# TXH-mercury/VALOR

Hardware: AMD Instinct MI355X
Metric: pretrain samples/sec (V+A+T clip) (higher is better)
Workload: dtype bf16

## Files before the change

### valor_amd/csrc/gemm8.hip

```cpp
#include "gemm_common.h"
#include <stdlib.h>

#define HT_BYTES 16384
#define BUF_BYTES (4 * HT_BYTES)
#define OFF_A0 0
#define OFF_A1 HT_BYTES
#define OFF_B0 (2 * HT_BYTES)
#define OFF_B1 (3 * HT_BYTES)

DEVINL bf16x8_t read_frag_tr8(const char* img, int off, int kk) {
    const char* a = img + off + kk * (32 * 256);
    s16x4_t lo = lds_read_tr4(a), hi = lds_read_tr4(a + 4 * 256);
    return __builtin_bit_cast(bf16x8_t, __builtin_shufflevector(lo, hi, 0, 1, 2, 3, 4, 5, 6, 7));
}

template <bool TA, bool TB, bool ASMTR, bool NTS = false, int SCHED = 0>
__global__ __launch_bounds__(512, 2) void gemm_8ph_kernel(GemmArgs p) {
    typedef bf16_t T;
    constexpr int BK = 64;
    extern __shared__ __attribute__((aligned(16))) char smem[];

    const int tid = threadIdx.x;
    const int lane = tid & 63;
    const int wave = __builtin_amdgcn_readfirstlane(tid >> 6);
    const int wm = wave >> 2, wn = wave & 3;
    const int fr = lane & 15, fg = lane >> 4;

    const int tiles_n = (p.N + 255) >> 8;
    const int tiles_m = (p.M + 255) >> 8;
    int logical, slice = 0;
    if (p.kslices > 1) {
        const int ntiles = tiles_m * tiles_n;
        const int item = xcd_remap(blockIdx.x, ntiles * p.kslices);
        slice = item / ntiles;
        logical = item - slice * ntiles;
    } else {
        logical = xcd_remap(blockIdx.x, tiles_m * tiles_n);
    }
    int tm = logical / tiles_n, tn = logical - tm * tiles_n;
    if (p.raster_g > 0 && p.kslices <= 1) {
        const int G = p.raster_g, per = G * tiles_m;
        const int grp = logical / per, w = logical - grp * per;
        const int gw = min(G, tiles_n - grp * G);
        tm = w / gw;
        tn = grp * G + (w - tm * gw);
    }
    const int m0 = tm << 8, n0 = tn << 8;

    const int nk_total = p.K / BK;
    int ks_begin = 0, ks_end = nk_total;
    if (p.kslices > 1) {
        ks_begin = slice * p.ksteps_per_slice;
        ks_end = ks_begin + p.ksteps_per_slice;
        if (ks_end > nk_total) ks_end = nk_total;
        if (ks_begin > nk_total) ks_begin = nk_total;
    }
    const int k_first = ks_begin * BK;

    f32x4_t acc[8][4];
#pragma unroll
    for (int i = 0; i < 8; ++i)
#pragma unroll
        for (int j = 0; j < 4; ++j) acc[i][j] = (f32x4_t){0.f, 0.f, 0.f, 0.f};

    const bool do_rs = TA && p.rowsum_out != nullptr && tn == 0;
    f32x4_t racc[2] = {(f32x4_t){0.f, 0.f, 0.f, 0.f}, (f32x4_t){0.f, 0.f, 0.f, 0.f}};
    const bf16x8_t ones = __builtin_bit_cast(bf16x8_t, (u32x4_t){0x3f803f80u, 0x3f803f80u, 0x3f803f80u, 0x3f803f80u});

    const rsrc_t rsA = make_rsrc(p.A, p.bytesA), rsB = make_rsrc(p.B, p.bytesB);
    int voA[2][2], voB[2][2];
    int stepA, stepB;
    {
        const int ldA_b = (int)(p.lda * 2), ldB_b = (int)(p.ldb * 2);
#pragma unroll
        for (int hf = 0; hf < 2; ++hf)
#pragma unroll
            for (int i = 0; i < 2; ++i) {
                const int pc = wave * 2 + i;
                if constexpr (!TA) {
                    const int r = pc * 8 + (lane >> 3), c = (lane & 7) ^ ((lane >> 3) & 7);
                    const int trow = hf * 128 + r;
                    voA[hf][i] = (m0 + trow) * ldA_b + (k_first + c * 8) * 2;
                } else {
                    const int k = pc * 4 + (lane >> 4), s = lane & 15;
                    const int ic = ((s - 2 * (k & 3) - 8 * ((k >> 3) & 1)) & 15) * 8;
                    const int trow = hf * 128 + ic;
                    voA[hf][i] = (k_first + k) * ldA_b + (m0 + trow) * 2;
                }
                if constexpr (!TB) {
                    const int r = pc * 8 + (lane >> 3), c = (lane & 7) ^ ((lane >> 3) & 7);
                    const int tcol = hf * 128 + r;
                    voB[hf][i] = (n0 + tcol) * ldB_b + (k_first + c * 8) * 2;
                } else {
                    const int k = pc * 4 + (lane >> 4), s = lane & 15;
                    const int ic = ((s - 2 * (k & 3) - 8 * ((k >> 3) & 1)) & 15) * 8;
                    const int tcol = hf * 128 + ic;
                    voB[hf][i] = (k_first + k) * ldB_b + (n0 + tcol) * 2;
                }
            }
        stepA = TA ? BK * ldA_b : BK * 2;
        stepB = TB ? BK * ldB_b : BK * 2;
    }
    auto issueA = [&](int hf, char* buf) {
        char* d = buf + (hf ? OFF_A1 : OFF_A0) + wave * 2048;
        glds16(rsA, d, voA[hf][0]);
        glds16(rsA, d + 1024, voA[hf][1]);
        voA[hf][0] += stepA; voA[hf][1] += stepA;
    };
    auto issueB = [&](int hf, char* buf) {
        char* d = buf + (hf ? OFF_B1 : OFF_B0) + wave * 2048;
        glds16(rsB, d, voB[hf][0]);
        glds16(rsB, d + 1024, voB[hf][1]);
        voB[hf][0] += stepB; voB[hf][1] += stepB;
    };

    int trA[4], trB[2];
    {
        const int base = (8 * fg + (fr >> 2)) * 256 + 8 * (fr & 1);
        const int rot = 2 * (fr >> 2) + 8 * (fg & 1);
#pragma unroll
        for (int i = 0; i < 4; ++i) trA[i] = base + 16 * ((2 * (wm * 4 + i) + ((fr >> 1) & 1) + rot) & 15);
#pragma unroll
        for (int i = 0; i < 2; ++i) trB[i] = base + 16 * ((2 * (wn * 2 + i) + ((fr >> 1) & 1) + rot) & 15);
    }
    bf16x8_t fa[4][2], fb0[2][2], fb1[2][2];
    TrPair pa[4][2], pb[2][2];
    auto readA = [&](const char* img) {
#pragma unroll
        for (int mt = 0; mt < 4; ++mt)
#pragma unroll
            for (int kk = 0; kk < 2; ++kk) {
                if constexpr (TA && ASMTR) tr_issue(pa[mt][kk], img + trA[mt] + kk * (32 * 256));
                else if constexpr (TA) fa[mt][kk] = read_frag_tr8(img, trA[mt], kk);
                else fa[mt][kk] = read_frag<T>(img, wm * 64 + mt * 16 + fr, kk * 4 + fg);
            }
    };
    auto readB = [&](const char* img, bf16x8_t (&fb)[2][2]) {
#pragma unroll
        for (int nt = 0; nt < 2; ++nt)
#pragma unroll
            for (int kk = 0; kk < 2; ++kk) {
                if constexpr (TB && ASMTR) tr_issue(pb[nt][kk], img + trB[nt] + kk * (32 * 256));
                else if constexpr (TB) fb[nt][kk] = read_frag_tr8(img, trB[nt], kk);
                else fb[nt][kk] = read_frag<T>(img, wn * 32 + nt * 16 + fr, kk * 4 + fg);
            }
    };
    auto fragA = [&]() {
        if constexpr (TA && ASMTR) {
            tr_wait8(pa);
#pragma unroll
            for (int mt = 0; mt < 4; ++mt)
#pragma unroll
                for (int kk = 0; kk < 2; ++kk) fa[mt][kk] = tr_frag(pa[mt][kk]);
        }
    };
    auto fragB = [&](bf16x8_t (&fb)[2][2]) {
        if constexpr (TB && ASMTR) {
            tr_wait4(pb);
#pragma unroll
            for (int nt = 0; nt < 2; ++nt)
#pragma unroll
                for (int kk = 0; kk < 2; ++kk) fb[nt][kk] = tr_frag(pb[nt][kk]);
        }
    };
#define QUADRANT(MH_, NH_, FB_)                                                                                   \
    do {                                                                                                          \
        __builtin_amdgcn_s_setprio(1);                                                                            \
        _Pragma("unroll") for (int kk = 0; kk < 2; ++kk)                                                          \
            _Pragma("unroll") for (int mt = 0; mt < 4; ++mt)                                                      \
                _Pragma("unroll") for (int nt = 0; nt < 2; ++nt)                                                  \
                    acc[(MH_) * 4 + mt][(NH_) * 2 + nt] = Mma<T>::mma(FB_[nt][kk], fa[mt][kk], acc[(MH_) * 4 + mt][(NH_) * 2 + nt]); \
        __builtin_amdgcn_s_setprio(0);                                                                            \
    } while (0)
#define ROWSUM(H_)                                                                                                \
    do {                                                                                                          \
        if (do_rs) {                                                                                              \
            _Pragma("unroll") for (int kk = 0; kk < 2; ++kk) {                                                    \
                const bf16x8_t f_ = wn == 0 ? fa[0][kk] : wn == 1 ? fa[1][kk] : wn == 2 ? fa[2][kk] : fa[3][kk];  \
                racc[H_] = Mma<T>::mma(ones, f_, racc[H_]);                                                       \
            }                                                                                                     \
        }                                                                                                         \
    } while (0)
#define LOAD_END()                                                                                                \
    do {                                                                                                          \
        asm volatile("s_waitcnt vmcnt(8)" ::: "memory");                                                          \
        __builtin_amdgcn_s_barrier();                                                                             \
        __builtin_amdgcn_sched_barrier(0);                                                                        \
    } while (0)
#define MATH_END()                                                                                                \
    do {                                                                                                          \
        __builtin_amdgcn_sched_barrier(0);                                                                        \
        __builtin_amdgcn_s_barrier();                                                                             \
        __builtin_amdgcn_sched_barrier(0);                                                                        \
    } while (0)

    char* const buf0 = smem;
    char* const buf1 = smem + BUF_BYTES;
    const int ntile = ks_end - ks_begin;

    if constexpr (SCHED == 1) {
        if (ntile > 0) {
            TrPair pb1[2][2];
            int oA[2][2], oB[2][2];
#pragma unroll
            for (int hf = 0; hf < 2; ++hf)
#pragma unroll
                for (int i = 0; i < 2; ++i) { oA[hf][i] = voA[hf][i]; oB[hf][i] = voB[hf][i]; }
            auto dmaA = [&](int hf, char* buf, int t, int i) {
                const rsrc_t rs = make_rsrc(p.A, t < ntile ? p.bytesA : 0u);
                glds16(rs, buf + (hf ? OFF_A1 : OFF_A0) + wave * 2048 + i * 1024, oA[hf][i]);
                oA[hf][i] += stepA; asm volatile("" : "+v"(oA[hf][i]));
            };
            auto dmaB = [&](int hf, char* buf, int t, int i) {
                const rsrc_t rs = make_rsrc(p.B, t < ntile ? p.bytesB : 0u);
                glds16(rs, buf + (hf ? OFF_B1 : OFF_B0) + wave * 2048 + i * 1024, oB[hf][i]);
                oB[hf][i] += stepB; asm volatile("" : "+v"(oB[hf][i]));
            };
#define RD_A(IMG_, MT_, KK_)                                                                                      \
    do {                                                                                                          \
        if constexpr (TA && ASMTR) tr_issue(pa[MT_][KK_], (IMG_) + trA[MT_] + (KK_) * (32 * 256));                \
        else if constexpr (TA) fa[MT_][KK_] = read_frag_tr8((IMG_), trA[MT_], (KK_));                             \
        else fa[MT_][KK_] = read_frag<T>((IMG_), wm * 64 + (MT_) * 16 + fr, (KK_) * 4 + fg);                      \
    } while (0)
#define RD_B(IMG_, NT_, KK_, FB_, PB_)                                                                            \
    do {                                                                                                          \
        if constexpr (TB && ASMTR) tr_issue(PB_[NT_][KK_], (IMG_) + trB[NT_] + (KK_) * (32 * 256));               \
        else if constexpr (TB) FB_[NT_][KK_] = read_frag_tr8((IMG_), trB[NT_], (KK_));                            \
        else FB_[NT_][KK_] = read_frag<T>((IMG_), wn * 32 + (NT_) * 16 + fr, (KK_) * 4 + fg);                     \
    } while (0)
#define PIN() __builtin_amdgcn_sched_barrier(0)
#define USE_A(KK_)                                                                                                \
    do {                                                                                                          \
        if constexpr (TA && ASMTR) {                                                                              \
            tr_wait_4(pa[0][KK_], pa[1][KK_], pa[2][KK_], pa[3][KK_]);                                            \
            _Pragma("unroll") for (int mt_ = 0; mt_ < 4; ++mt_) fa[mt_][KK_] = tr_frag(pa[mt_][KK_]);             \
            PIN();                                                                                                \
        }                                                                                                         \
    } while (0)
#define USE_B(KK_, FB_, PB_)                                                                                      \
    do {                                                                                                          \
        if constexpr (TB && ASMTR) {                                                                              \
            tr_wait_2(PB_[0][KK_], PB_[1][KK_]);                                                                  \
            _Pragma("unroll") for (int nt_ = 0; nt_ < 2; ++nt_) FB_[nt_][KK_] = tr_frag(PB_[nt_][KK_]);           \
            PIN();                                                                                                \
        }                                                                                                         \
    } while (0)
#define MF(MH_, NH_, MT_, NT_, KK_, FB_)                                                                          \
    acc[(MH_) * 4 + (MT_)][(NH_) * 2 + (NT_)] = Mma<T>::mma(FB_[NT_][KK_], fa[MT_][KK_], acc[(MH_) * 4 + (MT_)][(NH_) * 2 + (NT_)])
#define HALF8(MH_, NH_, KK_, FB_, X0, X1, X2, X3, X4, X5, X6, X7)                                               \
    do {                                                                                                          \
        MF(MH_, NH_, 0, 0, KK_, FB_); X0; PIN();                                                                  \
        MF(MH_, NH_, 0, 1, KK_, FB_); X1; PIN();                                                                  \
        MF(MH_, NH_, 1, 0, KK_, FB_); X2; PIN();                                                                  \
        MF(MH_, NH_, 1, 1, KK_, FB_); X3; PIN();                                                                  \
        MF(MH_, NH_, 2, 0, KK_, FB_); X4; PIN();                                                                  \
        MF(MH_, NH_, 2, 1, KK_, FB_); X5; PIN();                                                                  \
        MF(MH_, NH_, 3, 0, KK_, FB_); X6; PIN();                                                                  \
        MF(MH_, NH_, 3, 1, KK_, FB_); X7; PIN();                                                                  \
    } while (0)
#define ROWSUM1(H_, KK_)                                                                                          \
    do {                                                                                                          \
        if (do_rs) {                                                                                              \
            if (wn == 0) racc[H_] = Mma<T>::mma(ones, fa[0][KK_], racc[H_]);                                      \
            else if (wn == 1) racc[H_] = Mma<T>::mma(ones, fa[1][KK_], racc[H_]);                                 \
            else if (wn == 2) racc[H_] = Mma<T>::mma(ones, fa[2][KK_], racc[H_]);                                 \
            else racc[H_] = Mma<T>::mma(ones, fa[3][KK_], racc[H_]);                                              \
            PIN();                                                                                                \
        }                                                                                                         \
    } while (0)
#define WAIT_BARRIER(N_)                                                                                          \
    do {                                                                                                          \
        PIN();                                                                                                    \
        asm volatile("s_waitcnt vmcnt(" #N_ ")" ::: "memory");                                                    \
        __builtin_amdgcn_s_barrier();                                                                             \
        PIN();                                                                                                    \
    } while (0)
#pragma unroll
            for (int t = 0; t < 2; ++t) {
                char* const b = t ? buf1 : buf0;
                dmaA(0, b, t, 0); dmaA(0, b, t, 1); dmaB(0, b, t, 0); dmaB(0, b, t, 1);
                dmaB(1, b, t, 0); dmaB(1, b, t, 1); dmaA(1, b, t, 0); dmaA(1, b, t, 1);
            }
            WAIT_BARRIER(10);
            RD_B(buf0 + OFF_B1, 0, 0, fb1, pb1); RD_B(buf0 + OFF_B1, 1, 0, fb1, pb1); RD_B(buf0 + OFF_B1, 0, 1, fb1, pb1); RD_B(buf0 + OFF_B1, 1, 1, fb1, pb1);
            RD_B(buf0 + OFF_B0, 0, 0, fb0, pb); RD_B(buf0 + OFF_B0, 1, 0, fb0, pb);
            RD_A(buf0 + OFF_A0, 0, 0); RD_A(buf0 + OFF_A0, 1, 0); RD_A(buf0 + OFF_A0, 2, 0); RD_A(buf0 + OFF_A0, 3, 0);
            PIN();
            for (int rel = 0; rel < ntile; ++rel) {
                char* const cur = (rel & 1) ? buf1 : buf0;
                char* const nxt = (rel & 1) ? buf0 : buf1;
                USE_A(0); USE_B(0, fb0, pb);
                HALF8(0, 0, 0, fb0, RD_B(cur + OFF_B0, 0, 1, fb0, pb), RD_B(cur + OFF_B0, 1, 1, fb0, pb), RD_A(cur + OFF_A0, 0, 1), RD_A(cur + OFF_A0, 1, 1),
                      RD_A(cur + OFF_A0, 2, 1), RD_A(cur + OFF_A0, 3, 1), , );
                ROWSUM1(0, 0);
                USE_A(1); USE_B(1, fb0, pb);
                HALF8(0, 0, 1, fb0, , , , , , , , );
                ROWSUM1(0, 1);
                WAIT_BARRIER(8);
                USE_B(0, fb1, pb1); USE_B(1, fb1, pb1);
                HALF8(0, 1, 0, fb1, , dmaA(0, cur, rel + 2, 0), , dmaA(0, cur, rel + 2, 1), , dmaB(0, cur, rel + 2, 0), , dmaB(0, cur, rel + 2, 1));
                HALF8(0, 1, 1, fb1, RD_A(cur + OFF_A1, 0, 0), RD_A(cur + OFF_A1, 1, 0), RD_A(cur + OFF_A1, 2, 0), RD_A(cur + OFF_A1, 3, 0), , , , );
                USE_A(0);
                HALF8(1, 1, 0, fb1, RD_A(cur + OFF_A1, 0, 1), RD_A(cur + OFF_A1, 1, 1), RD_A(cur + OFF_A1, 2, 1), RD_A(cur + OFF_A1, 3, 1), , , , );
                ROWSUM1(1, 0);
                USE_A(1);
                HALF8(1, 1, 1, fb1, , , , dmaB(1, cur, rel + 2, 0), , , , dmaB(1, cur, rel + 2, 1));
                ROWSUM1(1, 1);
                WAIT_BARRIER(8);
                HALF8(1, 0, 0, fb0, RD_B(nxt + OFF_B1, 0, 0, fb1, pb1), RD_B(nxt + OFF_B1, 1, 0, fb1, pb1), RD_B(nxt + OFF_B1, 0, 1, fb1, pb1),
                      RD_B(nxt + OFF_B1, 1, 1, fb1, pb1), , dmaA(1, cur, rel + 2, 0), , dmaA(1, cur, rel + 2, 1));
                HALF8(1, 0, 1, fb0, RD_B(nxt + OFF_B0, 0, 0, fb0, pb), RD_B(nxt + OFF_B0, 1, 0, fb0, pb), RD_A(nxt + OFF_A0, 0, 0), RD_A(nxt + OFF_A0, 1, 0),
                      RD_A(nxt + OFF_A0, 2, 0), RD_A(nxt + OFF_A0, 3, 0), , );
            }
#undef RD_A
#undef RD_B
#undef PIN
#undef USE_A
#undef USE_B
#undef MF
#undef HALF8
#undef ROWSUM1
#undef WAIT_BARRIER
        }
    } else
    if (ntile > 0) {
        issueB(0, buf0); issueA(0, buf0); issueB(1, buf0); issueA(1, buf0); issueB(0, buf1); issueA(0, buf1);
        LOAD_END();
        if (wm == 1) __builtin_amdgcn_s_barrier();
        for (int rel = 0; rel < ntile; ++rel) {
            char* const cur = (rel & 1) ? buf1 : buf0;
            char* const nxt = (rel & 1) ? buf0 : buf1;
            readB(cur + OFF_B0, fb0);
            readA(cur + OFF_A0);
            issueB(1, nxt);
            LOAD_END();
            fragB(fb0); fragA();
            QUADRANT(0, 0, fb0);
            ROWSUM(0);
            MATH_END();
            readB(cur + OFF_B1, fb1);
            issueA(1, nxt);
            LOAD_END();
            fragB(fb1);
            QUADRANT(0, 1, fb1);
            MATH_END();
            readA(cur + OFF_A1);
            issueB(0, cur);
            LOAD_END();
            fragA();
            QUADRANT(1, 1, fb1);
            ROWSUM(1);
            MATH_END();
            issueA(0, cur);
            LOAD_END();
            QUADRANT(1, 0, fb0);
            MATH_END();
        }
        if (wm == 0) __builtin_amdgcn_s_barrier();
    }
    asm volatile("s_waitcnt vmcnt(0)" ::: "memory");
    __syncthreads();
#undef QUADRANT
#undef ROWSUM
#undef LOAD_END
#undef MATH_END
    if (do_rs && fg == 0) {
#pragma unroll
        for (int hh = 0; hh < 2; ++hh) {
            const int m = m0 + hh * 128 + wm * 64 + wn * 16 + fr;
            if (m < p.M) {
                if (p.kslices > 1) p.rowsum_ws[(int64_t)slice * p.M + m] = racc[hh][0];
                else rowsum_store<T>(p, m, racc[hh][0]);
            }
        }
    }

    if constexpr (!TA) if (p.fast_epi) {
        char* sB = smem;
        const int act = p.act & VALOR_ACT_MASK;
        const bool deriv = (p.act & VALOR_ACT_DERIV) != 0;
        auto write_tile = [&](bool apply_act) {
#pragma unroll
            for (int ni = 0; ni < 4; ++ni) {
                const int col = (ni >> 1) * 128 + wn * 32 + (ni & 1) * 16 + 4 * fg;
                const f32x4_t bias4 = load_bias4<T>(p, n0 + col);
#pragma unroll
                for (int mi = 0; mi < 8; ++mi) {
                    const int row = (mi >> 2) * 128 + wm * 64 + (mi & 3) * 16 + fr;
                    f32x4_t v = acc[mi][ni];
#pragma unroll
                    for (int r = 0; r < 4; ++r) v[r] = v[r] * p.alpha + bias4[r];
                    if (apply_act) {
                        float f[4] = {v[0], v[1], v[2], v[3]};
                        act_fwd_n<4>(act, f);
                        v = (f32x4_t){f[0], f[1], f[2], f[3]};
                    }
                    const u32x2_t w = {pack2_bf16(v[0], v[1]), pack2_bf16(v[2], v[3])};
                    *(u32x2_t*)(sB + row * 512 + (((col >> 3) ^ (row & 31)) << 4) + (fg & 1) * 8) = w;
                }
            }
        };
        auto read_tile = [&](T* dst) {
#pragma unroll 4
            for (int it = 0; it < 16; ++it) {
                const int ml = it * 16 + (tid >> 5), c = tid & 31;
                const u32x4_t val = *(const u32x4_t*)(sB + ml * 512 + ((c ^ (ml & 31)) << 4));
                const int m = m0 + ml, n = n0 + c * 8;
                if (m < p.M && n < p.N) store_out16<NTS>(dst + (int64_t)m * p.ldc + n, val);
            }
        };
        if (p.preact) {
            write_tile(false);
            __syncthreads();
            read_tile((T*)p.preact);
            __syncthreads();
        }
        write_tile(act != VALOR_ACT_NONE && !p.dact_aux);
        if (p.dact_aux || p.accumulate) {
            const bool dact = p.dact_aux != nullptr, accum = p.accumulate != 0;
            const T* src = dact ? (const T*)p.dact_aux : (const T*)p.C;
            const int64_t lds2 = dact ? p.ldaux : p.ldc;
            u32x4_t pre[16];
#pragma unroll
            for (int it = 0; it < 16; ++it) {
                const int m = m0 + it * 16 + (tid >> 5), n = n0 + (tid & 31) * 8;
                pre[it] = (u32x4_t){0u, 0u, 0u, 0u};
                if (m < p.M && n < p.N) pre[it] = *(const u32x4_t*)(src + (int64_t)m * lds2 + n);
            }
            __syncthreads();
            T* dst = (T*)p.C;
#pragma unroll
            for (int it = 0; it < 16; ++it) {
                const int ml = it * 16 + (tid >> 5), c = tid & 31;
                u32x4_t val = *(const u32x4_t*)(sB + ml * 512 + ((c ^ (ml & 31)) << 4));
                const int m = m0 + ml, n = n0 + c * 8;
                if (m < p.M && n < p.N) {
                    float f[8], x[8];
#pragma unroll
                    for (int q = 0; q < 4; ++q) { f[2 * q] = __uint_as_float(val[q] << 16); f[2 * q + 1] = __uint_as_float(val[q] & 0xffff0000u); }
#pragma unroll
                    for (int q = 0; q < 4; ++q) { x[2 * q] = __uint_as_float(pre[it][q] << 16); x[2 * q + 1] = __uint_as_float(pre[it][q] & 0xffff0000u); }
                    if (dact) {
                        if (deriv) {
#pragma unroll
                            for (int q = 0; q < 8; ++q) f[q] *= x[q];
                        } else {
                            act_bwd_mul_n<8>(act, f, x);
                        }
                        if (accum) {
                            const u32x4_t o = *(const u32x4_t*)(dst + (int64_t)m * p.ldc + n);
#pragma unroll
                            for (int q = 0; q < 4; ++q) { f[2 * q] += __uint_as_float(o[q] << 16); f[2 * q + 1] += __uint_as_float(o[q] & 0xffff0000u); }
                        }
                    } else {
#pragma unroll
                        for (int q = 0; q < 8; ++q) f[q] += x[q];
                    }
#pragma unroll
                    for (int q = 0; q < 4; ++q) val[q] = pack2_bf16(f[2 * q], f[2 * q + 1]);
                    store_out16<NTS>(dst + (int64_t)m * p.ldc + n, val);
                }
            }
            return;
        }
        __syncthreads();
        read_tile((T*)p.C);
        return;
    }

    float* sC = (float*)smem;
    float* wsl = p.kslices > 1 ? p.ws + (int64_t)slice * p.M * p.N : nullptr;
    const f32x4_t bias0 = load_bias4<T>(p, n0 + (tid & 31) * 8), bias1 = load_bias4<T>(p, n0 + (tid & 31) * 8 + 4);
#pragma unroll
    for (int pass = 0; pass < 2; ++pass) {
        if (pass) __syncthreads();
#pragma unroll
        for (int mt = 0; mt < 4; ++mt)
#pragma unroll
            for (int ni = 0; ni < 4; ++ni) {
                const int ml = wm * 64 + mt * 16 + fr;
                const int ch = ((ni >> 1) * 32 + wn * 8 + (ni & 1) * 4 + fg) ^ (ml & 7);
                *(f32x4_t*)(sC + ml * 256 + ch * 4) = acc[pass * 4 + mt][ni];
            }
        __syncthreads();
#pragma unroll 2
        for (int it = 0; it < 8; ++it) {
            const int ml = it * 16 + (tid >> 5);
            const int c8 = tid & 31;
            const f32x4_t v0 = *(const f32x4_t*)(sC + ml * 256 + (((2 * c8) ^ (ml & 7)) << 2));
            const f32x4_t v1 = *(const f32x4_t*)(sC + ml * 256 + (((2 * c8 + 1) ^ (ml & 7)) << 2));
            const int m = m0 + pass * 128 + ml, n = n0 + c8 * 8;
            if (wsl) {
                splitk_store8(p, slice, m, n, v0, v1);
            } else {
                epilogue_store8<true, NTS ? 1 : 0>(p, m, n, v0, v1, bias0, bias1);
            }
        }
    }
}

static int g_8ph_tr_asm = [] { const char* e = getenv("VALOR_GEMM_TR_ASM"); return e ? atoi(e) : 1; }();
extern "C" int valor_gemm_set_tr_asm(int v) {
    const int old = g_8ph_tr_asm;
    if (v >= 0) g_8ph_tr_asm = v;
    return old;
}

static int g_8ph_fast_epi = [] { const char* e = getenv("VALOR_GEMM_FAST_EPI"); return e ? atoi(e) : 1; }();
extern "C" int valor_gemm_set_fast_epilogue(int v) {
    const int old = g_8ph_fast_epi;
    if (v >= 0) g_8ph_fast_epi = v;
    return old;
}

static int g_8ph_sched = [] { const char* e = getenv("VALOR_GEMM_8PH_SCHED"); return e ? atoi(e) : 1000; }();
extern "C" int valor_gemm_set_8ph_sched(int v) {
    const int old = g_8ph_sched;
    if (v == 0 || v == 1 || v == 1000) g_8ph_sched = v;
    return old;
}

int gemm_tr_asm_now() { return GEMM_KNOB(tr_asm, g_8ph_tr_asm); }
int gemm_fast_epilogue_now() { return GEMM_KNOB(fast_epilogue, g_8ph_fast_epi); }

void launch_gemm_8ph(hipStream_t st, int transA, int transB, const GemmArgs& p_in) {
    GemmArgs p = p_in;
    const int fast_epi_ = gemm_fast_epilogue_now(), tr_asm_ = gemm_tr_asm_now();
    const bool light_dact = p.dact_aux && (p.act & VALOR_ACT_DERIV);
    const bool plainish = fast_epi_ >= 2 || (!p.preact && (!p.dact_aux || light_dact));
    p.fast_epi = fast_epi_ && plainish && !p.out_f32 && p.kslices <= 1 && (p.N & 7) == 0 && (p.ldc & 7) == 0 && !p.rowsum_out &&
                 (!p.dact_aux || (p.ldaux & 7) == 0) && !(p.dact_aux && p.preact) && !transA && !(p.preact && (p.act & VALOR_ACT_DERIV));
    const int tiles_m = (p.M + 255) / 256, tiles_n = (p.N + 255) / 256;
    const int tiles = tiles_m * tiles_n;
    p.raster_g = 0;
    if (p.kslices <= 1 && tiles_n > 1 && gemm_policy(4) != 0) {
        if (gemm_policy(4) != 1000) {
            p.raster_g = gemm_policy(4) < tiles_n ? gemm_policy(4) : 0;
        } else {
            const double panel = 256.0 * p.K * 2.0, a_bytes = (double)p.M * p.K * 2.0, rounds = tiles / 256.0;
            const double resident = 2.5 * 1048576.0;
            const int touched = tiles_n < 32 ? tiles_n : 32;
            double best = a_bytes + (tiles_n * panel <= resident ? 8.0 * tiles_n * panel : (rounds < 1.0 ? 1.0 : rounds) * 8.0 * touched * panel);
            for (int ng = 2; ng <= tiles_n; ++ng) {
                const int G = (tiles_n + ng - 1) / ng;
                if (G * panel > resident) continue;
                const double cost = ng * a_bytes + 8.0 * tiles_n * panel;
                if (cost < 0.9 * best) { best = cost; p.raster_g = G; }
            }
        }
    }
    const bool nts = !transA && !p.out_f32 && p.kslices <= 1 && (gemm_policy(5) == 1 || (gemm_policy(5) == 1000 && p.K <= 1024));
    p.st_mode = nts ? 1 : 0;
    dim3 grid(tiles * (p.kslices > 1 ? p.kslices : 1));
    const size_t lds = 2 * BUF_BYTES;
    int sched = GEMM_KNOB(sched_256, g_8ph_sched);
    if (sched == 1000) {
        const int ktiles = p.kslices > 1 ? p.ksteps_per_slice : p.K / 64;
        sched = transA ? (ktiles <= 48 ? 1 : 0) : (p.K >= 2048 ? 1 : 0);
    }
#define VALOR_8PH_LAUNCH(TA_, TB_, NTS_)                                                                        \
    do {                                                                                                        \
        static bool attr_set = false;                                                                           \
        constexpr bool kslow_ = TA_ || TB_;                                                                     \
        if (!attr_set) {                                                                                        \
            hipFuncSetAttribute((const void*)gemm_8ph_kernel<TA_, TB_, false, NTS_>, hipFuncAttributeMaxDynamicSharedMemorySize, (int)lds); \
            hipFuncSetAttribute((const void*)gemm_8ph_kernel<TA_, TB_, true, NTS_>, hipFuncAttributeMaxDynamicSharedMemorySize, (int)lds); \
            hipFuncSetAttribute((const void*)gemm_8ph_kernel<TA_, TB_, kslow_, NTS_, 1>, hipFuncAttributeMaxDynamicSharedMemorySize, (int)lds); \
            attr_set = true;                                                                                    \
        }                                                                                                       \
        if (sched == 1 && (tr_asm_ || !kslow_)) hipLaunchKernelGGL((gemm_8ph_kernel<TA_, TB_, kslow_, NTS_, 1>), grid, dim3(512), lds, st, p); \
        else if (tr_asm_ && kslow_) hipLaunchKernelGGL((gemm_8ph_kernel<TA_, TB_, true, NTS_>), grid, dim3(512), lds, st, p); \
        else hipLaunchKernelGGL((gemm_8ph_kernel<TA_, TB_, false, NTS_>), grid, dim3(512), lds, st, p);       \
    } while (0)
    if (!transA && !transB) { if (nts) VALOR_8PH_LAUNCH(false, false, true); else VALOR_8PH_LAUNCH(false, false, false); }
    else if (!transA && transB) { if (nts) VALOR_8PH_LAUNCH(false, true, true); else VALOR_8PH_LAUNCH(false, true, false); }
    else if (transA && !transB) VALOR_8PH_LAUNCH(true, false, false);
    else VALOR_8PH_LAUNCH(true, true, false);
#undef VALOR_8PH_LAUNCH
}
```

Baseline: 571.1.

## Add SCHED=2 GEMM k-loop with prefetched B fragments and split waitcnts

Adds a third main-loop schedule for the 8-phase 256x256 bf16 GEMM. It prefetches the next tile's B0 fragments at the end of each k-tile and unrolls the loop by two so the fragment registers alternate. It issues LDS reads with fine-grained lgkmcnt waits and raises wave priority with setprio around the MFMA blocks. For SCHED=2 the rowsum for the second half goes to the tn==1 tile, which spreads that extra work across tiles. The default auto policy now picks this schedule for several K and transpose shapes. Compile-time timestamp and ablation probes are also added but stay disabled by default. The extra fragment registers may raise register pressure.

```diff
diff --git a/valor_amd/csrc/gemm8.hip b/valor_amd/csrc/gemm8.hip
--- a/valor_amd/csrc/gemm8.hip
+++ b/valor_amd/csrc/gemm8.hip
@@ -8,6 +8,35 @@
 #define OFF_B0 (2 * HT_BYTES)
 #define OFF_B1 (3 * HT_BYTES)
 
+#ifdef G8_STAMP
+#define G8_MAXWG 2048
+__device__ uint64_t g8_stamp_buf[G8_MAXWG * 8 * 32];
+extern "C" int valor_gemm8_stamps(void* dst, int n_u64) {
+    if (n_u64 > G8_MAXWG * 8 * 32) n_u64 = G8_MAXWG * 8 * 32;
+    return hipMemcpyFromSymbol(dst, HIP_SYMBOL(g8_stamp_buf), (size_t)n_u64 * 8, 0, hipMemcpyDeviceToHost) == hipSuccess ? 0 : -1;
+}
+#define G8_STAMP_AT(i) stamp_[i] = __builtin_amdgcn_s_memtime()
+#define G8_HS(i) do { __builtin_amdgcn_sched_barrier(0); if (rel == 5) hs_[i] = __builtin_amdgcn_s_memtime(); __builtin_amdgcn_sched_barrier(0); } while (0)
+#else
+#define G8_STAMP_AT(i)
+#define G8_HS(i)
+#endif
+#if defined(G8_ABLATE) && (G8_ABLATE & 1)
+#define G8_DMA(...) do {} while (0)
+#else
+#define G8_DMA(...) __VA_ARGS__
+#endif
+#if defined(G8_ABLATE) && (G8_ABLATE & 2)
+#define G8_RD(...) do {} while (0)
+#else
+#define G8_RD(...) __VA_ARGS__
+#endif
+#if defined(G8_ABLATE) && (G8_ABLATE & 4)
+#define G8_RS_ON false
+#else
+#define G8_RS_ON true
+#endif
+
 DEVINL bf16x8_t read_frag_tr8(const char* img, int off, int kk) {
     const char* a = img + off + kk * (32 * 256);
     s16x4_t lo = lds_read_tr4(a), hi = lds_read_tr4(a + 4 * 256);
@@ -19,6 +48,10 @@
     typedef bf16_t T;
     constexpr int BK = 64;
     extern __shared__ __attribute__((aligned(16))) char smem[];
+#ifdef G8_STAMP
+    uint64_t stamp_[5] = {0, 0, 0, 0, 0}, rt_[2] = {0, 0}, hs_[9] = {0, 0, 0, 0, 0, 0, 0, 0, 0};
+    stamp_[0] = __builtin_amdgcn_s_memtime();
+#endif
 
     const int tid = threadIdx.x;
     const int lane = tid & 63;
@@ -63,7 +96,8 @@
 #pragma unroll
         for (int j = 0; j < 4; ++j) acc[i][j] = (f32x4_t){0.f, 0.f, 0.f, 0.f};
 
-    const bool do_rs = TA && p.rowsum_out != nullptr && tn == 0;
+    const bool do_rs = G8_RS_ON && TA && p.rowsum_out != nullptr && tn == 0;
+    const bool do_rs_hi = SCHED == 2 ? (G8_RS_ON && TA && p.rowsum_out != nullptr && tn == (tiles_n > 1 ? 1 : 0)) : do_rs;
     f32x4_t racc[2] = {(f32x4_t){0.f, 0.f, 0.f, 0.f}, (f32x4_t){0.f, 0.f, 0.f, 0.f}};
     const bf16x8_t ones = __builtin_bit_cast(bf16x8_t, (u32x4_t){0x3f803f80u, 0x3f803f80u, 0x3f803f80u, 0x3f803f80u});
 
@@ -322,53 +356,216 @@
 #undef ROWSUM1
 #undef WAIT_BARRIER
         }
-    } else
-    if (ntile > 0) {
+    } else if constexpr (SCHED == 2) {
+        if (ntile > 0) {
+            TrPair pb1[2][2];
+            auto rdA = [&](const char* img) {
+#pragma unroll
+                for (int kk = 0; kk < 2; ++kk)
+#pragma unroll
+                    for (int mt = 0; mt < 4; ++mt) {
+                        if constexpr (TA && ASMTR) tr_issue(pa[mt][kk], img + trA[mt] + kk * (32 * 256));
+                        else if constexpr (TA) fa[mt][kk] = read_frag_tr8(img, trA[mt], kk);
+                        else fa[mt][kk] = read_frag<T>(img, wm * 64 + mt * 16 + fr, kk * 4 + fg);
+                    }
+            };
+            auto rdB = [&](const char* img, bf16x8_t (&fb)[2][2], TrPair (&pq)[2][2]) {
+#pragma unroll
+                for (int kk = 0; kk < 2; ++kk)
+#pragma unroll
+                    for (int nt = 0; nt < 2; ++nt) {
+                        if constexpr (TB && ASMTR) tr_issue(pq[nt][kk], img + trB[nt] + kk * (32 * 256));
+                        else if constexpr (TB) fb[nt][kk] = read_frag_tr8(img, trB[nt], kk);
+                        else fb[nt][kk] = read_frag<T>(img, wn * 32 + nt * 16 + fr, kk * 4 + fg);
+                    }
+            };
+#define W_A(N_, KK_)                                                                                              \
+    do {                                                                                                          \
+        if constexpr (TA && ASMTR) {                                                                              \
+            asm volatile("s_waitcnt lgkmcnt(" #N_ ")" : TR_TIE(pa[0][KK_]), TR_TIE(pa[1][KK_]), TR_TIE(pa[2][KK_]), TR_TIE(pa[3][KK_])); \
+            _Pragma("unroll") for (int mt_ = 0; mt_ < 4; ++mt_) fa[mt_][KK_] = tr_frag(pa[mt_][KK_]);             \
+        }                                                                                                         \
+    } while (0)
+#define W_B(N_, KK_, PB_)                                                                                         \
+    do {                                                                                                          \
+        if constexpr (TB && ASMTR) asm volatile("s_waitcnt lgkmcnt(" #N_ ")" : TR_TIE(PB_[0][KK_]), TR_TIE(PB_[1][KK_])); \
+    } while (0)
+#define BV(FB_, PB_, NT_, KK_) (TB && ASMTR ? tr_frag(PB_[NT_][KK_]) : FB_[NT_][KK_])
+#define HALFQ(MH_, NH_, KK_, FB_, PB_)                                                                            \
+    _Pragma("unroll") for (int mt = 0; mt < 4; ++mt)                                                              \
+        _Pragma("unroll") for (int nt = 0; nt < 2; ++nt)                                                          \
+            acc[(MH_) * 4 + mt][(NH_) * 2 + nt] = Mma<T>::mma(BV(FB_, PB_, nt, KK_), fa[mt][KK_], acc[(MH_) * 4 + mt][(NH_) * 2 + nt])
+#define ROWSUM_H(H_, ON_)                                                                                         \
+    do {                                                                                                          \
+        if (ON_) {                                                                                                \
+            _Pragma("unroll") for (int kk = 0; kk < 2; ++kk) {                                                    \
+                const bf16x8_t f_ = wn == 0 ? fa[0][kk] : wn == 1 ? fa[1][kk] : wn == 2 ? fa[2][kk] : fa[3][kk];  \
+                racc[H_] = Mma<T>::mma(ones, f_, racc[H_]);                                                       \
+            }                                                                                                     \
+        }                                                                                                         \
+    } while (0)
+#define KTILE(REL_, FX_, PX_, FY_, PY_)                                                                           \
+    do {                                                                                                          \
+        const int rel = (REL_);                                                                                   \
+        char* const cur = (rel & 1) ? buf1 : buf0;                                                                \
+        char* const nxt = (rel & 1) ? buf0 : buf1;                                                                \
+        G8_HS(0);                                                                                                 \
+                                                                         \
+        G8_RD(rdA(cur + OFF_A0));                                                                                 \
+        G8_DMA(issueB(1, nxt));                                                                                   \
+        LOAD_END();                                                                                               \
+        G8_HS(1);                                                                                                 \
+        __builtin_amdgcn_s_setprio(1);                                                                            \
+        if constexpr (TA && ASMTR) { W_B(8, 0, PX_); W_B(8, 1, PX_); }       \
+        else { W_B(0, 0, PX_); W_B(0, 1, PX_); }                                                                  \
+        W_A(8, 0);                                                                                                \
+        HALFQ(0, 0, 0, FX_, PX_);                                                                                 \
+        W_A(0, 1);                                                                                                \
+        HALFQ(0, 0, 1, FX_, PX_);                                                                                 \
+        __builtin_amdgcn_s_setprio(0);                                                                            \
+        MATH_END();                                                                                               \
+        G8_HS(2);                                                                                                 \
+                                                        \
+        G8_RD(rdB(cur + OFF_B1, FY_, PY_));                                                                       \
+        G8_DMA(issueA(1, nxt));                                                                                   \
+        LOAD_END();                                                                                               \
+        G8_HS(3);                                                                                                 \
+        __builtin_amdgcn_s_setprio(1);                                                                            \
+        W_B(4, 0, PY_);                                                                                           \
+        HALFQ(0, 1, 0, FY_, PY_);                                                                                 \
+        W_B(0, 1, PY_);                                                                                           \
+        HALFQ(0, 1, 1, FY_, PY_);                                                                                 \
+        ROWSUM_H(0, do_rs);                                                                                       \
+        __builtin_amdgcn_s_setprio(0);                                                                            \
+        MATH_END();                                                                                               \
+        G8_HS(4);                                                                                                 \
+                                                                         \
+        G8_RD(rdA(cur + OFF_A1));                                                                                 \
+        G8_DMA(issueB(0, cur));                                                                                   \
+        LOAD_END();                                                                                               \
+        G8_HS(5);                                                                                                 \
+        __builtin_amdgcn_s_setprio(1);                                                                            \
+        W_A(8, 0);                                                                                                \
+        HALFQ(1, 1, 0, FY_, PY_);                                                                                 \
+        W_A(0, 1);                                                                                                \
+        HALFQ(1, 1, 1, FY_, PY_);                                                                                 \
+        __builtin_amdgcn_s_setprio(0);                                                                            \
+        MATH_END();                                                                                               \
+        G8_HS(6);                                                                                                 \
+                            \
+        if (rel + 1 < ntile) G8_RD(rdB(nxt + OFF_B0, FY_, PY_));                                                  \
+        G8_DMA(issueA(0, cur));                                                                                   \
+        LOAD_END();                                                                                               \
+        G8_HS(7);                                                                                                 \
+        __builtin_amdgcn_s_setprio(1);                                                                            \
+        HALFQ(1, 0, 0, FX_, PX_);                                                                                 \
+        HALFQ(1, 0, 1, FX_, PX_);                                                                                 \
+        ROWSUM_H(1, do_rs_hi);                                                                                    \
+        __builtin_amdgcn_s_setprio(0);                                                                            \
+        MATH_END();                                                                                               \
+        G8_HS(8);                                                                                                 \
+    } while (0)
+            issueB(0, buf0); issueA(0, buf0); issueB(1, buf0); issueA(1, buf0); issueB(0, buf1); issueA(0, buf1);
+            LOAD_END();
+            if (wm == 1) __builtin_amdgcn_s_barrier();
+            rdB(buf0 + OFF_B0, fb0, pb);
+            G8_STAMP_AT(1);
+#ifdef G8_STAMP
+            rt_[0] = __builtin_amdgcn_s_memrealtime();
+#endif
+            for (int r2 = 0; r2 < ntile; r2 += 2) {
+                KTILE(r2, fb0, pb, fb1, pb1);
+                if (r2 + 1 >= ntile) break;
+                KTILE(r2 + 1, fb1, pb1, fb0, pb);
+            }
+            if (wm == 0) __builtin_amdgcn_s_barrier();
+#undef W_A
+#undef W_B
+#undef BV
+#undef HALFQ
+#undef ROWSUM_H
+#undef KTILE
+        }
+    } else if (ntile > 0) {
         issueB(0, buf0); issueA(0, buf0); issueB(1, buf0); issueA(1, buf0); issueB(0, buf1); issueA(0, buf1);
         LOAD_END();
         if (wm == 1) __builtin_amdgcn_s_barrier();
+        G8_STAMP_AT(1);
+#ifdef G8_STAMP
+        rt_[0] = __builtin_amdgcn_s_memrealtime();
+#endif
         for (int rel = 0; rel < ntile; ++rel) {
             char* const cur = (rel & 1) ? buf1 : buf0;
             char* const nxt = (rel & 1) ? buf0 : buf1;
-            readB(cur + OFF_B0, fb0);
-            readA(cur + OFF_A0);
-            issueB(1, nxt);
+            G8_HS(0);
+            G8_RD(readB(cur + OFF_B0, fb0));
+            G8_RD(readA(cur + OFF_A0));
+            G8_DMA(issueB(1, nxt));
             LOAD_END();
+            G8_HS(1);
             fragB(fb0); fragA();
             QUADRANT(0, 0, fb0);
             ROWSUM(0);
             MATH_END();
-            readB(cur + OFF_B1, fb1);
-            issueA(1, nxt);
+            G8_HS(2);
+            G8_RD(readB(cur + OFF_B1, fb1));
+            G8_DMA(issueA(1, nxt));
             LOAD_END();
+            G8_HS(3);
             fragB(fb1);
             QUADRANT(0, 1, fb1);
             MATH_END();
-            readA(cur + OFF_A1);
-            issueB(0, cur);
+            G8_HS(4);
+            G8_RD(readA(cur + OFF_A1));
+            G8_DMA(issueB(0, cur));
             LOAD_END();
+            G8_HS(5);
             fragA();
             QUADRANT(1, 1, fb1);
             ROWSUM(1);
             MATH_END();
-            issueA(0, cur);
+            G8_HS(6);
+            G8_DMA(issueA(0, cur));
             LOAD_END();
+            G8_HS(7);
             QUADRANT(1, 0, fb0);
             MATH_END();
+            G8_HS(8);
         }
         if (wm == 0) __builtin_amdgcn_s_barrier();
     }
+    G8_STAMP_AT(2);
+#ifdef G8_STAMP
+    rt_[1] = __builtin_amdgcn_s_memrealtime();
+#endif
     asm volatile("s_waitcnt vmcnt(0)" ::: "memory");
     __syncthreads();
+    G8_STAMP_AT(3);
+#ifdef G8_STAMP
+    auto stamp_out = [&]() {
+        asm volatile("s_waitcnt vmcnt(0)" ::: "memory");
+        stamp_[4] = __builtin_amdgcn_s_memtime();
+        if (lane == 0 && blockIdx.x < G8_MAXWG) {
+            uint64_t* o = g8_stamp_buf + ((int64_t)blockIdx.x * 8 + wave) * 32;
+            for (int i = 0; i < 5; ++i) o[i] = stamp_[i];
+            o[5] = __builtin_amdgcn_s_getreg((31 << 11) | 4);
+            o[6] = __builtin_amdgcn_s_getreg((31 << 11) | 20);
+            o[7] = rt_[0]; o[8] = rt_[1]; o[9] = (uint64_t)ntile;
+            for (int i = 0; i < 9; ++i) o[10 + i] = hs_[i];
+        }
+    };
+#else
+    auto stamp_out = [&]() {};
+#endif
 #undef QUADRANT
 #undef ROWSUM
 #undef LOAD_END
 #undef MATH_END
-    if (do_rs && fg == 0) {
+    if ((do_rs || do_rs_hi) && fg == 0) {
 #pragma unroll
         for (int hh = 0; hh < 2; ++hh) {
             const int m = m0 + hh * 128 + wm * 64 + wn * 16 + fr;
-            if (m < p.M) {
+            if ((hh ? do_rs_hi : do_rs) && m < p.M) {
                 if (p.kslices > 1) p.rowsum_ws[(int64_t)slice * p.M + m] = racc[hh][0];
                 else rowsum_store<T>(p, m, racc[hh][0]);
             }
@@ -461,10 +658,12 @@
                     store_out16<NTS>(dst + (int64_t)m * p.ldc + n, val);
                 }
             }
+            stamp_out();
             return;
         }
         __syncthreads();
         read_tile((T*)p.C);
+        stamp_out();
         return;
     }
 
@@ -497,6 +696,7 @@
             }
         }
     }
+    stamp_out();
 }
 
 static int g_8ph_tr_asm = [] { const char* e = getenv("VALOR_GEMM_TR_ASM"); return e ? atoi(e) : 1; }();
@@ -516,8 +716,13 @@
 static int g_8ph_sched = [] { const char* e = getenv("VALOR_GEMM_8PH_SCHED"); return e ? atoi(e) : 1000; }();
 extern "C" int valor_gemm_set_8ph_sched(int v) {
     const int old = g_8ph_sched;
-    if (v == 0 || v == 1 || v == 1000) g_8ph_sched = v;
+    if (v == 0 || v == 1 || v == 2 || v == 1000 || v == 1001) g_8ph_sched = v;
     return old;
+}
+
+static bool gemm8_sched2_pick(int transA, int transB, int K, int ktiles) {
+    if (transA) return ktiles > 48;
+    return transB ? (K >= 1536 && K < 2048) : K >= 2048;
 }
 
 int gemm_tr_asm_now() { return GEMM_KNOB(tr_asm, g_8ph_tr_asm); }
@@ -554,9 +759,10 @@
     dim3 grid(tiles * (p.kslices > 1 ? p.kslices : 1));
     const size_t lds = 2 * BUF_BYTES;
     int sched = GEMM_KNOB(sched_256, g_8ph_sched);
-    if (sched == 1000) {
+    if (sched == 1000 || sched == 1001) {
         const int ktiles = p.kslices > 1 ? p.ksteps_per_slice : p.K / 64;
-        sched = transA ? (ktiles <= 48 ? 1 : 0) : (p.K >= 2048 ? 1 : 0);
+        const bool pick2 = sched == 1000 && gemm8_sched2_pick(transA, transB, p.K, ktiles);
+        sched = pick2 ? 2 : transA ? (ktiles <= 48 ? 1 : 0) : (p.K >= 2048 ? 1 : 0);
     }
 #define VALOR_8PH_LAUNCH(TA_, TB_, NTS_)                                                                        \
     do {                                                                                                        \
@@ -566,9 +772,11 @@
             hipFuncSetAttribute((const void*)gemm_8ph_kernel<TA_, TB_, false, NTS_>, hipFuncAttributeMaxDynamicSharedMemorySize, (int)lds); \
             hipFuncSetAttribute((const void*)gemm_8ph_kernel<TA_, TB_, true, NTS_>, hipFuncAttributeMaxDynamicSharedMemorySize, (int)lds); \
             hipFuncSetAttribute((const void*)gemm_8ph_kernel<TA_, TB_, kslow_, NTS_, 1>, hipFuncAttributeMaxDynamicSharedMemorySize, (int)lds); \
+            hipFuncSetAttribute((const void*)gemm_8ph_kernel<TA_, TB_, kslow_, NTS_, 2>, hipFuncAttributeMaxDynamicSharedMemorySize, (int)lds); \
             attr_set = true;                                                                                    \
         }                                                                                                       \
         if (sched == 1 && (tr_asm_ || !kslow_)) hipLaunchKernelGGL((gemm_8ph_kernel<TA_, TB_, kslow_, NTS_, 1>), grid, dim3(512), lds, st, p); \
+        else if (sched == 2 && (tr_asm_ || !kslow_)) hipLaunchKernelGGL((gemm_8ph_kernel<TA_, TB_, kslow_, NTS_, 2>), grid, dim3(512), lds, st, p); \
         else if (tr_asm_ && kslow_) hipLaunchKernelGGL((gemm_8ph_kernel<TA_, TB_, true, NTS_>), grid, dim3(512), lds, st, p); \
         else hipLaunchKernelGGL((gemm_8ph_kernel<TA_, TB_, false, NTS_>), grid, dim3(512), lds, st, p);       \
     } while (0)
```

Result: faster. 577.6 (median of 6 runs) (+1.1%).
